# arielmission-space/PAOS

Hardware: AMD Instinct MI355X
Metric: wavefronts/sec (4096^2 c128, 20-surface chain) + achieved HBM GB/s (higher is better)
Workload: dtype c128 (f64); 1 GPU; SYN20 20-surface chain (SURVEY 8d: 43 2-D FFTs per wavefront as the reference runs it), 4096x4096 fp64, walked 512-wavelength sweep, 32 wavefronts/GPU/step, PSFs stay in HBM; separable pass programs + ptp identities ([24] passes/wavefront, parity 1e-15..2e-14 vs oracle); grid=4096, batch_per_gpu=32, parallelism=wavefront-sharded x1, transport=none (single process), ranks_seen=1, launcher=none

## Files before the change

include/paos_hip.h:

```cpp
#ifndef PAOS_HIP_H
#define PAOS_HIP_H

#ifdef __cplusplus
extern "C" {
#endif

typedef struct paos_ctx paos_ctx;

enum { PAOS_OK = 0, PAOS_EINVAL = 1, PAOS_EHIP = 2, PAOS_EUNSUPPORTED = 3 };
enum { PAOS_F64 = 0, PAOS_F32 = 1 };
enum { PAOS_SHAPE_ELLIPSE = 0, PAOS_SHAPE_RECT = 1 };
enum { PAOS_KERNEL_PASS_ROWS = 0, PAOS_KERNEL_PASS_COLS = 1, PAOS_KERNEL_PASS_ANY = 2 };
enum { PAOS_PW_SIGN = 1, PAOS_PW_QPHASE_CENTRED = 2, PAOS_PW_QPHASE_NATURAL = 3, PAOS_PW_SCALE = 4,
       PAOS_PW_MASK = 5 };
enum { PAOS_PWF_MUL2PI = 1,
       PAOS_PWF_X_ONLY = 2, PAOS_PWF_Y_ONLY = 4 };
enum { PAOS_MAX_PW = 6 };
enum { PAOS_NORM_SLOTS = 64 };
enum { PAOS_WHAT_FIELD = 0, PAOS_WHAT_AMPLITUDE = 1, PAOS_WHAT_PHASE = 2, PAOS_WHAT_INTENSITY = 3 };

enum { PAOS_PHASE_STRIDE = 5 };
enum { PAOS_APERTURE_STRIDE = 8 };
enum { PAOS_ZERNIKE_HEAD = 8 };

// ... 68 lines not shown
int paos_phase_map_items(paos_ctx* ctx, const double* host_wfe, unsigned long long key, int n_items, const double* items,
                         const double* wl);
int paos_psd_screen(paos_ctx* ctx, const double* host_noise, const double* host_rough, const double* params,
                    unsigned long long key, double* host_out);
int paos_ptp(paos_ctx* ctx, const double* params);
int paos_stw(paos_ctx* ctx, const double* params, int inverse);
int paos_wts(paos_ctx* ctx, const double* params, int inverse);
int paos_focus_begin(paos_ctx* ctx);
int paos_focus_plane(paos_ctx* ctx, const double* params);
int paos_focus_end(paos_ctx* ctx);
enum { PAOS_OTF_MTF = 0, PAOS_OTF_COMPLEX = 1 };
int paos_otf_compute(paos_ctx* ctx);
int paos_otf_fetch(paos_ctx* ctx, int item, int what, void* host_out);
int paos_otf_cuts(paos_ctx* ctx, double* host_out);
int paos_blur_table(int n, double d, double sigma, double pixel, double* t);
enum { PAOS_BLUR_ITEM = 6 };
int paos_blur_apply(paos_ctx* ctx, const double* per_item);
enum { PAOS_EE_GIVEN = 0, PAOS_EE_CENTROID = 1, PAOS_EE_PEAK = 2 };
enum { PAOS_EE_ITEM = 4 };
enum { PAOS_EE_SUMMARY = 9 };
int paos_ee_compute(paos_ctx* ctx, int bins, int square, int centre_mode, const double* per_item);
int paos_ee_fetch(paos_ctx* ctx, double* summary, double* curves);
int paos_zoom_weights(int n, int s, double frac, double* w, int* carry);
enum { PAOS_ZOOM_PSF = 0, PAOS_ZOOM_FIELD = 1 };
int paos_zoom_compute(paos_ctx* ctx, int m, int s, const double* centres, int want_field);
int paos_zoom_tiles(int n, int batch, int m, int* pt_y, int* pt_x);
int paos_zoom_fetch(paos_ctx* ctx, int item, int what, void* host_out);
int paos_run_passes(paos_ctx* ctx, const paos_pass* passes, int n_passes, const double* blocks,
                    int n_blocks);
int paos_copy_yardstick(paos_ctx* ctx, int reps, double* ms_per_launch, double* bytes_per_launch);
int paos_record_set_stats(paos_ctx* ctx, unsigned long long* found, unsigned long long* rendered);
int paos_central_half_stats(paos_ctx* ctx, unsigned long long* central, unsigned long long* plain);
int paos_narrow_window_stats(paos_ctx* ctx, unsigned long long* narrow, unsigned long long* other);
int paos_frugal_built(int precision, int n, const int* record);
int paos_pass_builds(paos_ctx* ctx, int* records, int capacity, int* count);
int paos_deferred_stop_stats(paos_ctx* ctx, unsigned long long* rode, unsigned long long* settled);
int paos_ctx_set_pruning(paos_ctx* ctx, int on);
int paos_run_passes_live(paos_ctx* ctx, const paos_pass* passes, int n_passes, const double* blocks,
                         int n_blocks, const double* live_rows);
int paos_run_program(paos_ctx* ctx, const paos_pass* passes, int n_passes, const double* blocks, int n_blocks,
                     const paos_program_opts* opts);
int paos_zernike(paos_ctx* ctx, int nmax, int kdim, const double* table, const double* params,
                 int param_stride, double* host_wfe);
int paos_zernike_like(paos_ctx* ctx, int nmax, int kdim, const double* table, const double* params,
                      int param_stride, const double* same_as, double* host_wfe);


int paos_pupil_aperture(paos_ctx* ctx, int shape, const double* params);
int paos_pupil_upload(paos_ctx* ctx, int item, const double* host_weights);
int paos_zernike_gram(paos_ctx* ctx, int nmax, int kdim, const double* table, const double* params,
                      int param_stride, int K, const double* poly, int use_pupil, double* host_out);
int paos_zernike_pupil(paos_ctx* ctx, int nmax, int kdim, const double* table, const double* params,
                       int param_stride, double* host_wfe);

enum { PAOS_WF_UNIFORM = 0, PAOS_WF_INTENSITY = 1 };
enum { PAOS_WF_SUMMARY = 10 };
int paos_wavefront_fit(paos_ctx* ctx, int nmax, int kdim, const double* table, const double* params, int param_stride,
                       int K, const double* poly, int weight_mode, int use_pupil, const double* min_intensity);
int paos_wavefront_fetch(paos_ctx* ctx, double* summary, double* sums);

enum { PAOS_DETECTOR_GEOM = 6 };
enum { PAOS_DETECTOR_ITEM = 3 };
enum { PAOS_DETECTOR_SCRATCH_MIB = 512 };
int paos_detector_begin(paos_ctx* ctx, const double* geom);
int paos_detector_add(paos_ctx* ctx, const double* per_item);
int paos_detector_images(paos_ctx* ctx, const double* per_item, double* host_out);
// ... 10 lines not shown
```

paos_amd/_lib.py:

```python
import ctypes
import os
import threading
import weakref

import numpy as np

_HERE = os.path.dirname(os.path.abspath(__file__))
LIB_PATH = os.environ.get("PAOS_LIB") or os.path.join(_HERE, "libpaoship.so")

PAOS_F64, PAOS_F32 = 0, 1
SHAPE_ELLIPSE, SHAPE_RECT = 0, 1
WHAT_FIELD, WHAT_AMPLITUDE, WHAT_PHASE, WHAT_INTENSITY = 0, 1, 2, 3
KERNEL_PASS_ROWS, KERNEL_PASS_COLS, KERNEL_PASS_ANY = 0, 1, 2
PW_SIGN, PW_QPHASE_CENTRED, PW_QPHASE_NATURAL, PW_SCALE, PW_MASK = 1, 2, 3, 4, 5
PWF_MUL2PI = 1
PWF_X_ONLY, PWF_Y_ONLY = 2, 4
MAX_PW = 6
OTF_MTF, OTF_COMPLEX = 0, 1
EE_GIVEN, EE_CENTROID, EE_PEAK = 0, 1, 2
EE_ITEM, EE_SUMMARY, EE_MAX_BINS = 4, 9, 1024
WF_UNIFORM, WF_INTENSITY = 0, 1
WF_SUMMARY, WF_MAX_TERMS = 10, 63
ZOOM_PSF, ZOOM_FIELD = 0, 1
ZOOM_MAX_TABLES = 256
# ... 47 lines not shown
    "paos_norm2": (ctypes.c_int, [_c_ctx, _dbl_p]),
    "paos_norm2_enqueue": (ctypes.c_int, [_c_ctx, ctypes.POINTER(ctypes.c_int)]),
    "paos_norm2_fetch": (ctypes.c_int, [_c_ctx, ctypes.c_int, _dbl_p]),
    "paos_norm2_release": (ctypes.c_int, [_c_ctx, ctypes.c_int]),
    "paos_psf_metrics": (ctypes.c_int, [_c_ctx, ctypes.c_int, _dbl_p, ctypes.c_double, ctypes.c_double, _dbl_p]),
    "paos_phase": (ctypes.c_int, [_c_ctx, _dbl_p, ctypes.c_int]),
    "paos_phase_map": (ctypes.c_int, [_c_ctx, ctypes.c_int, _dbl_p, ctypes.c_double]),
    "paos_ptp": (ctypes.c_int, [_c_ctx, _dbl_p]),
    "paos_stw": (ctypes.c_int, [_c_ctx, _dbl_p, ctypes.c_int]),
    "paos_wts": (ctypes.c_int, [_c_ctx, _dbl_p, ctypes.c_int]),
    "paos_focus_begin": (ctypes.c_int, [_c_ctx]),
    "paos_focus_plane": (ctypes.c_int, [_c_ctx, _dbl_p]),
    "paos_focus_end": (ctypes.c_int, [_c_ctx]),
    "paos_otf_compute": (ctypes.c_int, [_c_ctx]),
    "paos_otf_fetch": (ctypes.c_int, [_c_ctx, ctypes.c_int, ctypes.c_int, ctypes.c_void_p]),
    "paos_otf_cuts": (ctypes.c_int, [_c_ctx, _dbl_p]),
    "paos_blur_table": (ctypes.c_int, [ctypes.c_int, ctypes.c_double, ctypes.c_double, ctypes.c_double, _dbl_p]),
    "paos_blur_apply": (ctypes.c_int, [_c_ctx, _dbl_p]),
    "paos_ee_compute": (ctypes.c_int, [_c_ctx, ctypes.c_int, ctypes.c_int, ctypes.c_int, _dbl_p]),
    "paos_ee_fetch": (ctypes.c_int, [_c_ctx, _dbl_p, _dbl_p]),
    "paos_wavefront_fit": (ctypes.c_int, [_c_ctx, ctypes.c_int, ctypes.c_int, _dbl_p, _dbl_p, ctypes.c_int, ctypes.c_int, _dbl_p,
                                          ctypes.c_int, ctypes.c_int, _dbl_p]),
    "paos_wavefront_fetch": (ctypes.c_int, [_c_ctx, _dbl_p, _dbl_p]),
    "paos_zoom_weights": (ctypes.c_int, [ctypes.c_int, ctypes.c_int, ctypes.c_double, _dbl_p, ctypes.POINTER(ctypes.c_int)]),
    "paos_zoom_compute": (ctypes.c_int, [_c_ctx, ctypes.c_int, ctypes.c_int, _dbl_p, ctypes.c_int]),
    "paos_zoom_fetch": (ctypes.c_int, [_c_ctx, ctypes.c_int, ctypes.c_int, ctypes.c_void_p]),
    "paos_zoom_tiles": (ctypes.c_int, [ctypes.c_int, ctypes.c_int, ctypes.c_int, ctypes.POINTER(ctypes.c_int),
                                       ctypes.POINTER(ctypes.c_int)]),
    "paos_run_passes": (ctypes.c_int, [_c_ctx, ctypes.POINTER(Pass), ctypes.c_int, _dbl_p, ctypes.c_int]),
    "paos_copy_yardstick": (ctypes.c_int, [_c_ctx, ctypes.c_int, _dbl_p, _dbl_p]),
    "paos_record_set_stats": (ctypes.c_int, [_c_ctx, ctypes.POINTER(ctypes.c_ulonglong), ctypes.POINTER(ctypes.c_ulonglong)]),
    "paos_central_half_stats": (ctypes.c_int, [_c_ctx, ctypes.POINTER(ctypes.c_ulonglong), ctypes.POINTER(ctypes.c_ulonglong)]),
    "paos_narrow_window_stats": (ctypes.c_int, [_c_ctx, ctypes.POINTER(ctypes.c_ulonglong), ctypes.POINTER(ctypes.c_ulonglong)]),
    "paos_frugal_built": (ctypes.c_int, [ctypes.c_int, ctypes.c_int, ctypes.POINTER(ctypes.c_int)]),
    "paos_pass_builds": (ctypes.c_int, [_c_ctx, ctypes.POINTER(ctypes.c_int), ctypes.c_int, ctypes.POINTER(ctypes.c_int)]),
    "paos_deferred_stop_stats": (ctypes.c_int, [_c_ctx, ctypes.POINTER(ctypes.c_ulonglong), ctypes.POINTER(ctypes.c_ulonglong)]),
    "paos_ctx_set_pruning": (ctypes.c_int, [_c_ctx, ctypes.c_int]),
    "paos_run_passes_live": (ctypes.c_int, [_c_ctx, ctypes.POINTER(Pass), ctypes.c_int, _dbl_p, ctypes.c_int, _dbl_p]),
    "paos_zernike": (ctypes.c_int, [_c_ctx, ctypes.c_int, ctypes.c_int, _dbl_p, _dbl_p, ctypes.c_int, _dbl_p]),
    "paos_psf_keep": (ctypes.c_int, [_c_ctx]),
    "paos_psf_keep_power": (ctypes.c_int, [_c_ctx, ctypes.POINTER(ctypes.c_int)]),
    "paos_psf_fetch": (ctypes.c_int, [_c_ctx, ctypes.c_int, _dbl_p]),
    "paos_host_alloc": (ctypes.c_int, [ctypes.c_ulonglong, ctypes.POINTER(ctypes.c_void_p)]),
    "paos_host_free": (ctypes.c_int, [ctypes.c_void_p]),
    "paos_export_pinned": (ctypes.c_int, [_c_ctx, ctypes.c_int, ctypes.c_int, ctypes.c_void_p]),
    "paos_start": (ctypes.c_int, [_c_ctx, ctypes.c_double, ctypes.c_double, ctypes.c_int, _dbl_p, _dbl_p]),
    "paos_pupil_aperture": (ctypes.c_int, [_c_ctx, ctypes.c_int, _dbl_p]),
    "paos_pupil_upload": (ctypes.c_int, [_c_ctx, ctypes.c_int, _dbl_p]),
    "paos_zernike_like": (ctypes.c_int, [_c_ctx, ctypes.c_int, ctypes.c_int, _dbl_p, _dbl_p, ctypes.c_int, _dbl_p, _dbl_p]),
    "paos_zernike_gram": (ctypes.c_int, [_c_ctx, ctypes.c_int, ctypes.c_int, _dbl_p, _dbl_p, ctypes.c_int,
                                         ctypes.c_int, _dbl_p, ctypes.c_int, _dbl_p]),
    "paos_zernike_pupil": (ctypes.c_int, [_c_ctx, ctypes.c_int, ctypes.c_int, _dbl_p, _dbl_p, ctypes.c_int, _dbl_p]),
    "paos_start_rows": (ctypes.c_int, [_c_ctx, ctypes.c_double, ctypes.c_double, ctypes.c_int, _dbl_p, _dbl_p, _dbl_p]),
    "paos_zero_outside_rows": (ctypes.c_int, [_c_ctx, _dbl_p]),
    "paos_phase_map_items": (ctypes.c_int, [_c_ctx, _dbl_p, ctypes.c_ulonglong, ctypes.c_int, _dbl_p, _dbl_p]),
    "paos_psd_screen": (ctypes.c_int, [_c_ctx, _dbl_p, _dbl_p, _dbl_p, ctypes.c_ulonglong, _dbl_p]),
    "paos_start_box": (ctypes.c_int, [_c_ctx, ctypes.c_double, ctypes.c_double, ctypes.c_int, _dbl_p, _dbl_p, _dbl_p, _dbl_p]),
    "paos_start_zernike_box": (ctypes.c_int, [_c_ctx, ctypes.c_double, ctypes.c_double, ctypes.c_int, _dbl_p, _dbl_p, _dbl_p, _dbl_p,
                                              ctypes.c_int, ctypes.c_int, _dbl_p, _dbl_p, ctypes.c_int, ctypes.POINTER(ctypes.c_int)]),
    "paos_zero_outside_box": (ctypes.c_int, [_c_ctx, _dbl_p, _dbl_p]),
    "paos_norm2_enqueue_box": (ctypes.c_int, [_c_ctx, _dbl_p, _dbl_p, _dbl_p, ctypes.POINTER(ctypes.c_int)]),
    "paos_norm2_enqueue_rows": (ctypes.c_int, [_c_ctx, _dbl_p, ctypes.POINTER(ctypes.c_int)]),
    "paos_norm2_enqueue_rows_like": (ctypes.c_int, [_c_ctx, _dbl_p, _dbl_p, ctypes.POINTER(ctypes.c_int)]),
    "paos_run_program": (ctypes.c_int, [_c_ctx, ctypes.POINTER(Pass), ctypes.c_int, _dbl_p, ctypes.c_int,
                                        ctypes.POINTER(ProgramOpts)]),
    "paos_detector_begin": (ctypes.c_int, [_c_ctx, _dbl_p]),
# ... 557 lines not shown
        ctr = None if centres is None else zoom_centres(centres, self.batch, self.n)
        zoom_check(size, oversample, self.n)
        self._check(self._lib.paos_zoom_compute(self._ctx, int(size), int(oversample), _dptr(ctr) if ctr is not None else None,
                                                1 if field else 0), "paos_zoom_compute")
        self._zoom_size = int(size)

    def zoom_fetch(self, item=0, what="psf"):
        if what not in ("psf", "field"):
            raise ValueError(f"what must be 'psf' or 'field', got {what!r}")
        m = getattr(self, "_zoom_size", 1)
        out = np.empty((m, m), dtype=np.float64 if what == "psf" else np.complex128)
        self._check(self._lib.paos_zoom_fetch(self._ctx, int(item), ZOOM_PSF if what == "psf" else ZOOM_FIELD,
                                              out.ctypes.data_as(ctypes.c_void_p)), "paos_zoom_fetch")
        return out

    def copy_yardstick(self, reps=10):
        ms, nbytes = ctypes.c_double(0.0), ctypes.c_double(0.0)
        self._check(self._lib.paos_copy_yardstick(self._ctx, int(reps), ctypes.byref(ms), ctypes.byref(nbytes)),
                    "paos_copy_yardstick")
        return ms.value, nbytes.value

    def record_set_stats(self):
        found, rendered = ctypes.c_ulonglong(0), ctypes.c_ulonglong(0)
        self._check(self._lib.paos_record_set_stats(self._ctx, ctypes.byref(found), ctypes.byref(rendered)),
                    "paos_record_set_stats")
        return int(found.value), int(rendered.value)

    def central_half_stats(self):
        central, plain = ctypes.c_ulonglong(0), ctypes.c_ulonglong(0)
        self._check(self._lib.paos_central_half_stats(self._ctx, ctypes.byref(central), ctypes.byref(plain)),
                    "paos_central_half_stats")
        return int(central.value), int(plain.value)

    def pass_builds(self, capacity=64):
        count = ctypes.c_int(0)
        buf = (ctypes.c_int * (9 * capacity))()
        self._check(self._lib.paos_pass_builds(self._ctx, buf, capacity, ctypes.byref(count)), "paos_pass_builds")
        if count.value > capacity:
            return self.pass_builds(count.value)
        return [tuple(buf[9 * i:9 * i + 9]) for i in range(count.value)]

    def deferred_stop_stats(self):
        rode, settled = ctypes.c_ulonglong(0), ctypes.c_ulonglong(0)
        self._check(self._lib.paos_deferred_stop_stats(self._ctx, ctypes.byref(rode), ctypes.byref(settled)),
                    "paos_deferred_stop_stats")
        return int(rode.value), int(settled.value)

    def set_pruning(self, on):
        self._check(self._lib.paos_ctx_set_pruning(self._ctx, 1 if on else 0), "paos_ctx_set_pruning")

    def run_passes(self, passes, blocks, live_rows=None, rows_stale=False, final_intensity=False, live_cols=None):
        b = np.ascontiguousarray(blocks, dtype=np.float64)
        if b.ndim != 3 or b.shape[1:] != (self.batch, PHASE_STRIDE):
            raise ValueError("blocks must be [n_blocks][batch][5]")
        arr = (Pass * len(passes))()
        for dst, src in zip(arr, passes):
            dst.axis, dst.fft1, dst.fft2 = src["axis"], src.get("fft1", -1), src.get("fft2", -1)
            for name in ("pre", "mid", "post"):
                ops = src.get(name, ())
                if len(ops) > MAX_PW:
                    raise ValueError("too many operators in one pass slot")
                setattr(dst, "n_" + name, len(ops))
                lst = getattr(dst, name)
                for i, (kind, flags, block) in enumerate(ops):
                    lst[i].kind, lst[i].flags, lst[i].block = kind, flags, block
        if rows_stale or final_intensity:
# ... 104 lines not shown
```

paos_amd/csrc/context.hip:

```cpp
#include "host.h"

#include <cmath>
#include <complex>
#include <cstdio>
#include <cstring>
#include <mutex>
#include <set>
#include <utility>

namespace {

thread_local std::string g_err;

}

int fail(paos_ctx* c, int code, const std::string& msg) {
  if (c) c->err = msg;
  g_err = msg;
  return code;
}

namespace {

bool dump_arena() {
// ... 358 lines not shown
  if (n > capacity) return fail(c, PAOS_EINVAL, "profile buffer too small");
  for (int i = 0; i < n; ++i) lines_out[i] = (size_t)i < c->prof_lines.size() ? c->prof_lines[i] : 0.0;
  *count = n;
  return PAOS_OK;
}

int paos_profile_end(paos_ctx* c, int* launches, double* total_ms) {
  return profile_end(c, launches, total_ms, nullptr, nullptr);
}

int paos_profile_end_split(paos_ctx* c, int* launches, double* total_ms, int* pruned_launches, double* pruned_ms) {
  if (!pruned_launches || !pruned_ms) return fail(c, PAOS_EINVAL, "null argument");
  return profile_end(c, launches, total_ms, pruned_launches, pruned_ms);
}

int paos_ctx_destroy(paos_ctx* c) {
  if (!c) return PAOS_OK;
  (void)hipSetDevice(c->device);
  if (c->stream) (void)hipStreamSynchronize(c->stream);
  for (hipEvent_t e : c->prof_events) (void)hipEventDestroy(e);
  if (c->field) (void)hipFree(c->field);
  if (c->tw) (void)hipFree(c->tw);
  if (c->staging) (void)hipFree(c->staging);
  if (c->tables) (void)hipFree(c->tables);
  if (c->mask) (void)hipFree(c->mask);
  if (c->metric_partial) (void)hipFree(c->metric_partial);
  if (c->metric_out) (void)hipFree(c->metric_out);
  if (c->metric_host) (void)hipHostFree(c->metric_host);
  for (auto& ms : c->mask_sets) {
    if (ms.lines) (void)hipFree(ms.lines);
    if (ms.vals) (void)hipFree(ms.vals);
  }
  if (c->mask_overflow) (void)hipFree(c->mask_overflow);
  if (c->partial) (void)hipFree(c->partial);
  if (c->norm2) (void)hipFree(c->norm2);
  if (c->norm2_host) (void)hipHostFree(c->norm2_host);
  if (c->psf) (void)hipFree(c->psf);
  if (c->focus_spec) (void)hipFree(c->focus_spec);
  if (c->otf_spec) (void)hipFree(c->otf_spec);
  if (c->otf_cuts) (void)hipFree(c->otf_cuts);
  if (c->zoom_t) (void)hipFree(c->zoom_t);
  if (c->zoom_psf) (void)hipFree(c->zoom_psf);
  if (c->zoom_field) (void)hipFree(c->zoom_field);
  if (c->zoom_tabs) (void)hipFree(c->zoom_tabs);
  if (c->map_dev) (void)hipFree(c->map_dev);
  if (c->psd_scratch) (void)hipFree(c->psd_scratch);
  if (c->start_norm2) (void)hipFree(c->start_norm2);
  if (c->start_partial) (void)hipFree(c->start_partial);
  if (c->psd_bad) (void)hipFree(c->psd_bad);
  if (c->pow_partial) (void)hipFree(c->pow_partial);
  if (c->dyn_scale) (void)hipFree(c->dyn_scale);
  if (c->ptab) (void)hipFree(c->ptab);
  if (c->psf_partial) (void)hipFree(c->psf_partial);
  if (c->det_img) (void)hipFree(c->det_img);
  if (c->det_rows) (void)hipFree(c->det_rows);
  if (c->det_out) (void)hipFree(c->det_out);
  if (c->ee_buf) (void)hipFree(c->ee_buf);
  if (c->wf_buf) (void)hipFree(c->wf_buf);
  for (int i = 0; i < 2; ++i) {
    if (c->bounce[i]) (void)hipHostFree(c->bounce[i]);
    if (c->bounce_ev[i]) (void)hipEventDestroy(c->bounce_ev[i]);
  }
  if (c->arena.host) (void)hipHostFree(c->arena.host);
  if (c->arena.dev) (void)hipFree(c->arena.dev);
  for (int k = 0; k < kArenaSlabs; ++k)
    if (c->arena.fence[k]) (void)hipEventDestroy(c->arena.fence[k]);
// ... 34 lines not shown
  HIPCHK(c, hipStreamSynchronize(c->stream));
  c->norm_busy[ticket] = false;
  std::memcpy(host_out, c->norm2_host + (size_t)ticket * c->batch, (size_t)c->batch * sizeof(double));
  return check_mask_overflow(c);
}

int paos_norm2_release(paos_ctx* c, int ticket) {
  if (!c || ticket < 0 || ticket >= kNormSlots) return fail(c, PAOS_EINVAL, "bad ticket");
  c->norm_busy[ticket] = false;
  return PAOS_OK;
}

int paos_record_set_stats(paos_ctx* c, unsigned long long* found, unsigned long long* rendered) {
  if (!c || !found || !rendered) return fail(c, PAOS_EINVAL, "bad record-set request");
  *found = c->mask_hits;
  *rendered = c->mask_rendered;
  return PAOS_OK;
}

int paos_central_half_stats(paos_ctx* c, unsigned long long* central, unsigned long long* plain) {
  if (!c || !central || !plain) return fail(c, PAOS_EINVAL, "bad central-half request");
  *central = c->central_launches;
  *plain = c->plain_launches;
  return PAOS_OK;
}

int paos_narrow_window_stats(paos_ctx* c, unsigned long long* narrow, unsigned long long* other) {
  if (!c || !narrow || !other) return fail(c, PAOS_EINVAL, "bad narrow-window request");
  *narrow = c->narrow_launches;
  *other = c->other_launches;
  return PAOS_OK;
}

int paos_deferred_stop_stats(paos_ctx* c, unsigned long long* rode, unsigned long long* settled) {
  if (!c || !rode || !settled) return fail(c, PAOS_EINVAL, "bad deferred-stop request");
  *rode = c->deferred_rode;
  *settled = c->deferred_settled;
  return PAOS_OK;
}

int paos_ctx_set_pruning(paos_ctx* c, int on) {
  if (!c) return fail(c, PAOS_EINVAL, "null context");
  c->prune = on != 0;
  return PAOS_OK;
}

}
```

paos_amd/csrc/host.h:

```cpp
#pragma once
#include "../../include/paos_hip.h"

#include <hip/hip_runtime.h>

#include <cstdlib>
#include <string>
#include <type_traits>
#include <vector>

#include "arena_layout.h"
#include "frugal_pass.h"
#include "pass_records.h"

using namespace paos;

#ifndef PAOS_BR
#define PAOS_BR 4
#endif
#ifndef PAOS_PAD_BLOCKS
#define PAOS_PAD_BLOCKS 3
#endif
inline constexpr int BR = PAOS_BR;
#ifndef PAOS_F32_BR
#define PAOS_F32_BR 8
// ... 74 lines not shown
  bool ee_computed = false, ee_valid = false;
  double* wf_buf = nullptr;
  size_t wf_bytes = 0;
  int wf_pairs = 0;
  bool wf_fitted = false;
  void* bounce[2] = {nullptr, nullptr};
  hipEvent_t bounce_ev[2] = {nullptr, nullptr};
  void* field = nullptr;
  void* tw = nullptr;
  void* staging = nullptr;
  cx<double>* tables = nullptr;
  double* mask = nullptr;
  double* metric_partial = nullptr;
  double* metric_out = nullptr;
  double* metric_host = nullptr;
  struct MaskSet {
    MaskLine* lines = nullptr;
    double* vals = nullptr;
    std::vector<double> key;
    unsigned long long used = 0;
    int line_lo = 0, line_hi = 0;
  };
  static constexpr int kMaskSets = 8;
  MaskSet mask_sets[kMaskSets];
  unsigned long long mask_clock = 0;
  unsigned long long mask_hits = 0, mask_rendered = 0;
  size_t lds_pad = 0;
  bool central_half = true;
  unsigned long long central_launches = 0, plain_launches = 0;
  bool narrow_windows = true;
  unsigned long long narrow_launches = 0, other_launches = 0;
  std::vector<int> pass_builds;
  int* mask_overflow = nullptr;
  double* partial = nullptr;
  double* norm2 = nullptr;
  double* norm2_host = nullptr;
  bool prune = true;
  int norm_slot = 0;
  bool norm_busy[64] = {};
  int nparts = 0;
  Arena arena;
  std::string err;
  int prof_kind = -1;
  std::vector<hipEvent_t> prof_events;
  std::vector<int> prof_tags;
  int prof_next_tag = 0;
  double prof_next_bytes = 0.0;
  std::vector<double> prof_bytes;
  double prof_next_lines = 0.0;
  std::vector<double> prof_lines;
  size_t prof_used = 0;
};

#pragma GCC visibility push(hidden)

int fail(paos_ctx* c, int code, const std::string& msg);

#define HIPCHK(c, call)                                                                     \
  do {                                                                                      \
    hipError_t e_ = (call);                                                                 \
    if (e_ != hipSuccess)                                                                   \
      return fail((c), PAOS_EHIP,                                                           \
                  std::string(#call) + ": " + hipGetErrorString(e_) + " (" __FILE__ ":" +   \
                      std::to_string(__LINE__) + ")");                                      \
  } while (0)

// ... 129 lines not shown
```

paos_amd/csrc/paos_hip.hip:

```cpp
#include "host.h"

#include <algorithm>
#include <cmath>
#include <cstring>

#include "item_groups.h"
#include "pointwise.h"

namespace {

int pw_blocks(const paos_ctx* c) {
  const size_t total = (size_t)c->item_stride;
  size_t b = (total + kPwThreads - 1) / kPwThreads;
  return (int)(b < 2048 ? b : 2048);
}

__global__ void dyn_scale_set_kernel(double* dyn, const double* norm2, const double* enable, int batch) {
  const int i = blockIdx.x * blockDim.x + threadIdx.x;
  if (i < batch) dyn[i] = (!enable || enable[i] != 0.0) ? 1.0 / sqrt(norm2[i]) : 1.0;
}
__global__ void dyn_scale_reset_kernel(double* dyn, int batch) {
  const int i = blockIdx.x * blockDim.x + threadIdx.x;
  if (i < batch) dyn[i] = 1.0;
}
// ... 8 lines not shown
}

}

int dyn_scale_reset(paos_ctx* c) {
  hipLaunchKernelGGL(dyn_scale_reset_kernel, dim3((c->batch + 255) / 256), dim3(256), 0, c->stream, c->dyn_scale, c->batch);
  HIPCHK(c, hipGetLastError());
  c->dyn_pending = false;
  return PAOS_OK;
}

int settle_scale(paos_ctx* c, bool field_is_overwritten) {
  if (!c->dyn_pending) return PAOS_OK;
  ++c->deferred_settled;
  if (!field_is_overwritten) {
    const dim3 grid(pw_blocks(c), c->batch), block(kPwThreads);
    dispatch_layout(c, [&](auto t, auto) {
      using T = decltype(t);
      hipLaunchKernelGGL(scale_by_kernel<T>, grid, block, 0, c->stream, (cx<T>*)c->field, c->dyn_scale, c->item_stride);
    });
  }
  return dyn_scale_reset(c);
}

static_assert(kMaskRenders == kMaskJobs, "a call's renderings go out in one launch per shape");
int render_mask_records(paos_ctx* c, const MaskRender* renders, int count) {
  MaskJobs jobs{};
  for (int j = 0; j < count; ++j) {
    const MaskRender& r = renders[j];
    const paos_ctx::MaskSet& ms = c->mask_sets[r.set];
    jobs.job[j] = MaskJob{r.params, r.shared, ms.lines, ms.vals, r.axis, r.line0, r.line_end, r.shapes};
  }
  jobs.batch_stride = c->batch * (int)FP_STRIDE; jobs.param_stride = (int)FP_STRIDE; jobs.n = c->n; jobs.overflow = c->mask_overflow;
  {
    const int mode = mask_render_mode();
    jobs.windows = mode != 0 ? 1 : 0;
    jobs.pairs = mode >= 2 ? mode - 1 : 0;
    jobs.rect_blocks = mask_rect_blocks() ? 1 : 0;
  }
  int widest = 0, shapes = 0;
  for (int j = 0; j < count; ++j) {
    widest = std::max(widest, jobs.job[j].line_end - jobs.job[j].line0);
    shapes |= jobs.job[j].shapes;
  }
  const dim3 block(256);
  const int per_wg = 4 * (jobs.pairs >= 2 ? 4 : (jobs.pairs ? 2 : 1));
  if (shapes & 1) hipLaunchKernelGGL(mask_lines_kernel<0>, dim3((widest + per_wg - 1) / per_wg, c->batch, count), block, 0, c->stream, jobs);
  const int rect_per_wg = 4 * (jobs.rect_blocks ? 64 : 1);
  if (shapes & 2) hipLaunchKernelGGL(mask_lines_kernel<1>, dim3((widest + rect_per_wg - 1) / rect_per_wg, c->batch, count), block, 0, c->stream, jobs);
  HIPCHK(c, hipGetLastError());
  return PAOS_OK;
}

int render_mask_weights(paos_ctx* c, const double* ap) {
  if (!c->mask) HIPCHK(c, hipMalloc(&c->mask, (size_t)c->batch * c->item_stride * sizeof(double)));
  const dim3 grid(pw_blocks(c), c->batch), block(kPwThreads);
  const double* ap2 = ap + (size_t)c->batch * FP_STRIDE;
  dispatch_layout(c, [&](auto t, auto br) {
    using T = decltype(t);
    constexpr int BRV = decltype(br)::value;
    hipLaunchKernelGGL((aperture_kernel<T, BRV, Lay<T>::BC, 0>), grid, block, 0, c->stream, (cx<T>*)nullptr, ap, ap2, FP_STRIDE, c->n, c->pitch, c->item_stride, c->mask, 1);
    hipLaunchKernelGGL((aperture_kernel<T, BRV, Lay<T>::BC, 1>), grid, block, 0, c->stream, (cx<T>*)nullptr, ap, ap2, FP_STRIDE, c->n, c->pitch, c->item_stride, c->mask, 1);
  });
  HIPCHK(c, hipGetLastError());
  return PAOS_OK;
}

int pointwise_pass(paos_ctx* c, const PassArgs& a) {
  const dim3 grid(pw_blocks(c), c->batch), block(kPwThreads);
  dispatch_layout(c, [&](auto t, auto br) {
    hipLaunchKernelGGL((pointwise_kernel<decltype(t), decltype(br)::value, Lay<decltype(t)>::BC>), grid, block, 0, c->stream, a, c->n);
  });
  HIPCHK(c, hipGetLastError());
  return PAOS_OK;
}

namespace {

const char* const kPhaseMapOverflow = "the phase argument 2 pi w / wl of the map's largest value is not finite";
bool phase_map_argument_finite(double wmax, double wl) { return std::isfinite((6.283185307179586 * wmax) / wl); }
// ... 951 lines not shown
```

paos_amd/csrc/passes.hip:

```cpp
#include "frugal_launch.h"

#include <algorithm>
#include <cmath>
#include <cstdio>
#include <cstring>

#include "pass_program.h"
#include "phase_tables.h"

namespace {

int check_ops(paos_ctx* c, const paos_pw_op* ops, int count, int n_blocks) {
  if (count < 0 || count > PAOS_MAX_PW) return fail(c, PAOS_EINVAL, "too many pointwise operators in a pass");
  for (int o = 0; o < count; ++o) {
    if (ops[o].kind < PAOS_PW_SIGN || ops[o].kind > PAOS_PW_MASK) return fail(c, PAOS_EINVAL, "unknown pointwise operator");
    if (ops[o].block < 0 || ops[o].block >= n_blocks) return fail(c, PAOS_EINVAL, "operator block index out of range");
    if (ops[o].kind == PAOS_PW_MASK && ops[o].block + 1 >= n_blocks) return fail(c, PAOS_EINVAL, "an aperture operator needs two parameter blocks");
  }
  return PAOS_OK;
}

bool use_tables() {
  static const bool on = env_is("PAOS_PHASE_TABLES", '1');
  return on;
}

bool use_frugal() {
  static const bool on = !env_is("PAOS_NO_FRUGAL", '1');
  return on;
}

bool frugal_sizes(const paos_ctx* c) {
  return use_frugal() && c->n >= (c->precision == PAOS_F64 ? 1024 : 2048);
}

int ensure_mask_store(paos_ctx* c) {
  if (!c->mask_overflow) {
    HIPCHK(c, hipMalloc(&c->mask_overflow, sizeof(int)));
    HIPCHK(c, hipMemsetAsync(c->mask_overflow, 0, sizeof(int), c->stream));
  }
  return PAOS_OK;
}

int assign_mask_set(paos_ctx* c, const paos_pass& p, LoweredPass& lp, const double* blocks) {
  std::vector<double> key;
  key.reserve((size_t)2 * c->batch * FP_STRIDE + c->batch + 3);
  key.push_back((double)p.axis);
  key.push_back((double)(mask_render_mode() + (mask_rect_blocks() ? 0 : 8)));
  const double* ap = blocks + (size_t)lp.mask_block * c->batch * FP_STRIDE;
  key.insert(key.end(), ap, ap + (size_t)2 * c->batch * FP_STRIDE);
  key.insert(key.end(), lp.mask_shared.begin(), lp.mask_shared.end());
  int hit = -1, victim = 0;
  for (int k = 0; k < paos_ctx::kMaskSets; ++k) {
    const paos_ctx::MaskSet& ms = c->mask_sets[k];
    if (!ms.key.empty() && ms.key.size() == key.size() && !std::memcmp(ms.key.data(), key.data(), key.size() * sizeof(double))) hit = k;
    if (ms.used < c->mask_sets[victim].used) victim = k;
  }
  const int k = hit >= 0 ? hit : victim;
  paos_ctx::MaskSet& ms = c->mask_sets[k];
  if (!ms.lines) {
    for (paos_ctx::MaskSet& m2 : c->mask_sets) {
      if (m2.lines) continue;
      HIPCHK(c, hipMalloc(&m2.lines, (size_t)c->batch * c->n * sizeof(MaskLine)));
      HIPCHK(c, hipMalloc(&m2.vals, (size_t)c->batch * c->n * 2 * kMaskW * sizeof(double)));
    }
  }
  ms.used = ++c->mask_clock;
  lp.mask_set = k;
  lp.mask_render = hit < 0;
  lp.mask_shapes = 0;
  for (int it = 0; it < c->batch; ++it) {
    const double* a1 = ap + (size_t)it * FP_STRIDE;
// ... 391 lines not shown
  return take_power_ticket(c, c->psf_partial, c->n / frugal_tile_lines(c, r.passes[r.n_passes - 1].axis), nullptr, final_ticket);
}

int run_passes_impl(paos_ctx* c, const paos_pass* passes, int n_passes, const double* blocks, int n_blocks,
                    const double* entry_rows, bool entry_stale, int* final_ticket, int final_mode, const double* entry_cols) {
  int rc = validate_program(c, passes, n_passes, blocks, n_blocks, final_ticket);
  if (rc) return rc;
  final_mode = final_ticket ? (final_mode == 2 ? 2 : 1) : 0;
  ProgramRun r(c, passes, n_passes, blocks, n_blocks);
  if ((rc = open_batch(r)) || (rc = lower_and_assign_sets(r)) || (rc = settle_stop(r))) return rc;
  plan_lines(r, entry_rows, entry_stale, entry_cols);
  if (entry_stale && entry_rows && entry_zero_first(r.d, r.pruned, r.low, entry_rows, entry_cols)) {
    if ((rc = entry_cols ? zero_outside_box(c, entry_rows, entry_cols) : zero_outside_rows(c, entry_rows))) return rc;
  }
  if ((rc = prepare_store(r, final_mode)) || (rc = batch_renderings(r)) || (rc = plan_and_stage_launches(r))) return rc;
  if ((rc = r.ab.commit())) return rc;
  for (size_t at = 0; at < r.renderings.size(); at += kMaskRenders)
    if ((rc = render_mask_records(c, r.renderings.data() + at, (int)std::min<size_t>(kMaskRenders, r.renderings.size() - at)))) return rc;
  if ((rc = launch_staged_tables(c, r.staged)) || (rc = launch_chunks(r))) return rc;
  return final_mode ? hand_out_ticket(r, final_mode, final_ticket) : PAOS_OK;
}

}

int run_passes(paos_ctx* c, const paos_pass* passes, int n_passes, const double* blocks, int n_blocks, const double* entry_rows,
               bool entry_stale, int* final_ticket, int final_mode, const double* entry_cols) {
  const int rc = arena_settled(c, run_passes_impl(c, passes, n_passes, blocks, n_blocks, entry_rows, entry_stale, final_ticket, final_mode, entry_cols));
  if (rc != PAOS_OK && c) forget_mask_sets(c);
  return rc;
}

int mask_render_mode() {
  if (env_is("PAOS_MASK_SCAN", '1')) return 0;
  return env_is("PAOS_MASK_PAIRS", '0') ? 1 : (env_is("PAOS_MASK_PAIRS", '1') ? 2 : 3);
}
bool mask_rect_blocks() {
  return !env_is("PAOS_MASK_RECT_BLOCKS", '0');
}

namespace {

struct Program {
  std::vector<paos_pass> passes;
  std::vector<double> blocks;
  int batch;
  explicit Program(int b) : batch(b) {}
  int add_block(const double* src, double v1, double v2, double v3, double v4, bool copy) {
    const int id = (int)(blocks.size() / ((size_t)batch * FP_STRIDE));
    for (int i = 0; i < batch; ++i) {
      const double* s = src + (size_t)i * FP_STRIDE;
      if (copy) blocks.insert(blocks.end(), s, s + FP_STRIDE);
      else blocks.insert(blocks.end(), {s[FP_ENABLE], v1, v2, v3, v4});
    }
    return id;
  }
  paos_pass& add_pass(int axis, int fft1, int fft2) {
    paos_pass p{};
    p.axis = axis; p.fft1 = fft1; p.fft2 = fft2;
    passes.push_back(p);
    return passes.back();
  }
};
void push(paos_pw_op* list, int& count, int kind, int block, int flags = 0) { list[count++] = {kind, flags, block}; }

enum FftOp { OP_PTP, OP_STW, OP_WTS };

int fft_op(paos_ctx* c, FftOp op, const double* params, int inverse) {
// ... 103 lines not shown
```

paos_amd/csrc/pointwise.h:

```cpp
#pragma once
#include "frugal_pass.h"
#include "item_window.h"
#include "pointwise_shared.h"

namespace paos {

template <typename T>
__global__ void fill_kernel(cx<T>* f, size_t total, T re, T im) {
  size_t i = (size_t)blockIdx.x * blockDim.x + threadIdx.x;
  for (; i < total; i += (size_t)gridDim.x * blockDim.x) f[i] = {re, im};
}

template <typename T>
__global__ void rmw_copy_kernel(cx<T>* f, size_t total) {
  size_t i = (size_t)blockIdx.x * blockDim.x + threadIdx.x;
  for (; i < total; i += (size_t)gridDim.x * blockDim.x) {
    cx<T> v = f[i];
    asm volatile("" : "+v"(v.x), "+v"(v.y));
    f[i] = v;
  }
}

template <typename T, int BR, int BC>
__global__ void import_kernel(cx<T>* f, const cx<double>* staged, int n, unsigned pitch) {
  const size_t total = (size_t)pitch * (n / BR);
  size_t m = (size_t)blockIdx.x * blockDim.x + threadIdx.x;
  for (; m < total; m += (size_t)gridDim.x * blockDim.x) {
    int r, c;
    if (!layout_unmap<BR, BC>(m, n, pitch, r, c)) continue;
    const cx<double> v = staged[(size_t)r * n + c];
    f[m] = {(T)v.x, (T)v.y};
  }
}

template <typename T, int BR, int BC>
__global__ void export_kernel(const cx<T>* f, double* out, int n, unsigned pitch, int what) {
// ... 816 lines not shown
  }
  const int len0 = e.p1 - e.p0, len1 = e.p3 - e.p2i;
  for (unsigned long long todo = in_lines; todo; todo &= todo - 1) {
    const int k = (int)__ffsll((long long)todo) - 1;
    double* vout = jb.vals + ((size_t)item * n + (first + k)) * (2 * kMaskW);
    for (int j = lane; j < len0; j += 64) vout[j] = prof[j];
    for (int j = lane; j < len1; j += 64) vout[kMaskW + j] = prof[kMaskW + j];
  }
}

template <int SHAPE>
__global__ void __launch_bounds__(kMaskWaves * 64) mask_lines_kernel(MaskJobs jobs) {
  const MaskJob& jb = jobs.job[blockIdx.z];
  if (!(jb.shapes & (1 << SHAPE))) return;
  const int item = blockIdx.y;
  if (jb.shared[item] != 0.0) return;
  const int lane = threadIdx.x & 63;
  const int wave = blockIdx.x * (blockDim.x >> 6) + (threadIdx.x >> 6);
  if (SHAPE == 1 && jobs.rect_blocks != 0) {
    __shared__ double prof[kMaskWaves][2 * kMaskW];
    mask_rect_block_render(jobs, jb, item, jb.line0 + 64 * wave, lane, prof[threadIdx.x >> 6]);
    return;
  }
  const int per = SHAPE == 0 && jobs.pairs != 0 ? (jobs.pairs >= 2 ? 4 : 2) : 1;
  const int first = jb.line0 + per * wave;
  if (first >= jb.line_end || first >= jobs.n) return;
  if (SHAPE == 0 && per == 4 && mask_multi_render<4>(jobs, jb, item, first, lane)) return;
  for (int f = first; f < first + per; f += 2) {
    if (SHAPE == 0 && per >= 2 && mask_multi_render<2>(jobs, jb, item, f, lane)) continue;
    for (int line = f; line < f + (per >= 2 ? 2 : 1); ++line) {
      if (SHAPE == 0 && jobs.windows != 0 && mask_multi_render<1>(jobs, jb, item, line, lane)) continue;
      mask_line_render<SHAPE>(jobs, jb, item, line, lane);
    }
  }
}


template <int NMAXC>
__device__ __forceinline__ double zernike_wfe(const double* table, const double* coef_c, const double* coef_s, int nmax, int kdim,
                                              double x, double y, double rr, double rho, bool origin_y, double co, double so) {
  double wfe = 0.0;
  double c1 = 1.0, s1 = 0.0;
  if (rr > 0.0) {
    c1 = (origin_y ? y : x) / rr;
    s1 = (origin_y ? x : y) / rr;
  }
  const double cr = c1 * co - s1 * so, sr = s1 * co + c1 * so;
  const double xj = 1.0 - 2.0 * rho * rho;
  double rho_pow = 1.0, cm = 1.0, sm = 0.0;
  auto order = [&](int am, int k_end) __attribute__((always_inline)) {
    double pkm1 = 0.0, pk = 1.0;
    for (int k = 0; k <= k_end; ++k) {
      if (k > 0) {
        const double* abc = table + ((size_t)am * kdim + k) * 3;
        const double pn = (abc[0] * xj + abc[1]) * pk - abc[2] * pkm1;
        pkm1 = pk;
        pk = pn;
      }
      const size_t ci = (size_t)am * kdim + k;
      wfe += (rho_pow * pk) * (coef_c[ci] * cm + coef_s[ci] * sm);
    }
    rho_pow *= rho;
    const double cn = cm * cr - sm * sr;
    sm = sm * cr + cm * sr;
    cm = cn;
  };
// ... 313 lines not shown
```

Before: 2496 wavefronts/s.

## Render ellipse mask records per 64-line block with shared undecided-pixel list

Adds a default-on mask_blocks_kernel in which each wavefront handles 64 lines at once. Each lane classifies its line's edge-window pixels as in, out or undecided. The undecided pixels from all lanes are compacted into a shared-memory list so that the expensive per-pixel weight evaluation runs lane-parallel across the whole block instead of per line. Lines that overflow the list or have no fitting window fall back to the existing per-line renderers. Device atomic counters and a stats API are added, which brings extra atomics, LDS use and complexity.

```diff
diff --git a/include/paos_hip.h b/include/paos_hip.h
--- a/include/paos_hip.h
+++ b/include/paos_hip.h
@@ -124,6 +124,7 @@
 int paos_record_set_stats(paos_ctx* ctx, unsigned long long* found, unsigned long long* rendered);
 int paos_central_half_stats(paos_ctx* ctx, unsigned long long* central, unsigned long long* plain);
 int paos_narrow_window_stats(paos_ctx* ctx, unsigned long long* narrow, unsigned long long* other);
+int paos_record_block_stats(paos_ctx* ctx, unsigned long long* out);
 int paos_frugal_built(int precision, int n, const int* record);
 int paos_pass_builds(paos_ctx* ctx, int* records, int capacity, int* count);
 int paos_deferred_stop_stats(paos_ctx* ctx, unsigned long long* rode, unsigned long long* settled);
diff --git a/paos_amd/_lib.py b/paos_amd/_lib.py
--- a/paos_amd/_lib.py
+++ b/paos_amd/_lib.py
@@ -103,6 +103,7 @@
     "paos_record_set_stats": (ctypes.c_int, [_c_ctx, ctypes.POINTER(ctypes.c_ulonglong), ctypes.POINTER(ctypes.c_ulonglong)]),
     "paos_central_half_stats": (ctypes.c_int, [_c_ctx, ctypes.POINTER(ctypes.c_ulonglong), ctypes.POINTER(ctypes.c_ulonglong)]),
     "paos_narrow_window_stats": (ctypes.c_int, [_c_ctx, ctypes.POINTER(ctypes.c_ulonglong), ctypes.POINTER(ctypes.c_ulonglong)]),
+    "paos_record_block_stats": (ctypes.c_int, [_c_ctx, ctypes.POINTER(ctypes.c_ulonglong)]),
     "paos_frugal_built": (ctypes.c_int, [ctypes.c_int, ctypes.c_int, ctypes.POINTER(ctypes.c_int)]),
     "paos_pass_builds": (ctypes.c_int, [_c_ctx, ctypes.POINTER(ctypes.c_int), ctypes.c_int, ctypes.POINTER(ctypes.c_int)]),
     "paos_deferred_stop_stats": (ctypes.c_int, [_c_ctx, ctypes.POINTER(ctypes.c_ulonglong), ctypes.POINTER(ctypes.c_ulonglong)]),
@@ -726,6 +727,11 @@
                     "paos_central_half_stats")
         return int(central.value), int(plain.value)
 
+    def record_block_stats(self):
+        out = (ctypes.c_ulonglong * 3)()
+        self._check(self._lib.paos_record_block_stats(self._ctx, out), "paos_record_block_stats")
+        return int(out[0]), int(out[1]), int(out[2])
+
     def pass_builds(self, capacity=64):
         count = ctypes.c_int(0)
         buf = (ctypes.c_int * (9 * capacity))()
diff --git a/paos_amd/csrc/context.hip b/paos_amd/csrc/context.hip
--- a/paos_amd/csrc/context.hip
+++ b/paos_amd/csrc/context.hip
@@ -414,6 +414,7 @@
     if (ms.vals) (void)hipFree(ms.vals);
   }
   if (c->mask_overflow) (void)hipFree(c->mask_overflow);
+  if (c->block_stats) (void)hipFree(c->block_stats);
   if (c->partial) (void)hipFree(c->partial);
   if (c->norm2) (void)hipFree(c->norm2);
   if (c->norm2_host) (void)hipHostFree(c->norm2_host);
@@ -514,6 +515,15 @@
   return PAOS_OK;
 }
 
+int paos_record_block_stats(paos_ctx* c, unsigned long long* out) {
+  if (!c || !out) return fail(c, PAOS_EINVAL, "bad record-block request");
+  out[0] = out[1] = out[2] = 0ull;
+  if (!c->block_stats) return PAOS_OK;
+  HIPCHK(c, hipStreamSynchronize(c->stream));
+  HIPCHK(c, hipMemcpy(out, c->block_stats, 3 * sizeof(unsigned long long), hipMemcpyDeviceToHost));
+  return PAOS_OK;
+}
+
 int paos_deferred_stop_stats(paos_ctx* c, unsigned long long* rode, unsigned long long* settled) {
   if (!c || !rode || !settled) return fail(c, PAOS_EINVAL, "bad deferred-stop request");
   *rode = c->deferred_rode;
diff --git a/paos_amd/csrc/host.h b/paos_amd/csrc/host.h
--- a/paos_amd/csrc/host.h
+++ b/paos_amd/csrc/host.h
@@ -130,6 +130,7 @@
   unsigned long long narrow_launches = 0, other_launches = 0;
   std::vector<int> pass_builds;
   int* mask_overflow = nullptr;
+  unsigned long long* block_stats = nullptr;
   double* partial = nullptr;
   double* norm2 = nullptr;
   double* norm2_host = nullptr;
diff --git a/paos_amd/csrc/paos_hip.hip b/paos_amd/csrc/paos_hip.hip
--- a/paos_amd/csrc/paos_hip.hip
+++ b/paos_amd/csrc/paos_hip.hip
@@ -64,12 +64,10 @@
     jobs.job[j] = MaskJob{r.params, r.shared, ms.lines, ms.vals, r.axis, r.line0, r.line_end, r.shapes};
   }
   jobs.batch_stride = c->batch * (int)FP_STRIDE; jobs.param_stride = (int)FP_STRIDE; jobs.n = c->n; jobs.overflow = c->mask_overflow;
-  {
-    const int mode = mask_render_mode();
-    jobs.windows = mode != 0 ? 1 : 0;
-    jobs.pairs = mode >= 2 ? mode - 1 : 0;
-    jobs.rect_blocks = mask_rect_blocks() ? 1 : 0;
-  }
+  const int mode = mask_render_mode();
+  jobs.windows = mode != 0 ? 1 : 0;
+  jobs.pairs = mode >= 2 ? std::min(mode, 3) - 1 : 0;
+  jobs.rect_blocks = mask_rect_blocks() ? 1 : 0;
   int widest = 0, shapes = 0;
   for (int j = 0; j < count; ++j) {
     widest = std::max(widest, jobs.job[j].line_end - jobs.job[j].line0);
@@ -77,7 +75,11 @@
   }
   const dim3 block(256);
   const int per_wg = 4 * (jobs.pairs >= 2 ? 4 : (jobs.pairs ? 2 : 1));
-  if (shapes & 1) hipLaunchKernelGGL(mask_lines_kernel<0>, dim3((widest + per_wg - 1) / per_wg, c->batch, count), block, 0, c->stream, jobs);
+  constexpr int block_per_wg = kMaskBlockLines * kMaskWaves;
+  if ((shapes & 1) && mode == 4)
+    hipLaunchKernelGGL(mask_blocks_kernel, dim3((widest + block_per_wg - 1) / block_per_wg, c->batch, count), block, 0, c->stream, jobs, c->block_stats);
+  else if (shapes & 1)
+    hipLaunchKernelGGL(mask_lines_kernel<0>, dim3((widest + per_wg - 1) / per_wg, c->batch, count), block, 0, c->stream, jobs);
   const int rect_per_wg = 4 * (jobs.rect_blocks ? 64 : 1);
   if (shapes & 2) hipLaunchKernelGGL(mask_lines_kernel<1>, dim3((widest + rect_per_wg - 1) / rect_per_wg, c->batch, count), block, 0, c->stream, jobs);
   HIPCHK(c, hipGetLastError());
diff --git a/paos_amd/csrc/passes.hip b/paos_amd/csrc/passes.hip
--- a/paos_amd/csrc/passes.hip
+++ b/paos_amd/csrc/passes.hip
@@ -38,6 +38,10 @@
   if (!c->mask_overflow) {
     HIPCHK(c, hipMalloc(&c->mask_overflow, sizeof(int)));
     HIPCHK(c, hipMemsetAsync(c->mask_overflow, 0, sizeof(int), c->stream));
+  }
+  if (!c->block_stats) {
+    HIPCHK(c, hipMalloc(&c->block_stats, 3 * sizeof(unsigned long long)));
+    HIPCHK(c, hipMemsetAsync(c->block_stats, 0, 3 * sizeof(unsigned long long), c->stream));
   }
   return PAOS_OK;
 }
@@ -495,7 +499,9 @@
 
 int mask_render_mode() {
   if (env_is("PAOS_MASK_SCAN", '1')) return 0;
-  return env_is("PAOS_MASK_PAIRS", '0') ? 1 : (env_is("PAOS_MASK_PAIRS", '1') ? 2 : 3);
+  if (env_is("PAOS_MASK_PAIRS", '0')) return 1;
+  if (env_is("PAOS_MASK_PAIRS", '1')) return 2;
+  return env_is("PAOS_MASK_BLOCKS", '0') ? 3 : 4;
 }
 bool mask_rect_blocks() {
   return !env_is("PAOS_MASK_RECT_BLOCKS", '0');
diff --git a/paos_amd/csrc/pointwise.h b/paos_amd/csrc/pointwise.h
--- a/paos_amd/csrc/pointwise.h
+++ b/paos_amd/csrc/pointwise.h
@@ -2,6 +2,7 @@
 #include "frugal_pass.h"
 #include "item_window.h"
 #include "pointwise_shared.h"
+#include "record_blocks.h"
 
 namespace paos {
 
@@ -884,6 +885,111 @@
       if (SHAPE == 0 && jobs.windows != 0 && mask_multi_render<1>(jobs, jb, item, line, lane)) continue;
       mask_line_render<SHAPE>(jobs, jb, item, line, lane);
     }
+  }
+}
+
+constexpr int kMaskBlockLines = 64;
+__global__ void __launch_bounds__(kMaskWaves * 64) mask_blocks_kernel(MaskJobs jobs, unsigned long long* stats) {
+  const MaskJob& jb = jobs.job[blockIdx.z];
+  if (!(jb.shapes & 1)) return;
+  const int item = blockIdx.y;
+  if (jb.shared[item] != 0.0) return;
+  const int lane = threadIdx.x & 63, wv = threadIdx.x >> 6;
+  const int n = jobs.n, axis = jb.axis;
+  const int first = jb.line0 + kMaskBlockLines * (blockIdx.x * kMaskWaves + wv);
+  if (first >= jb.line_end || first >= n) return;
+  MaskLineGeom<0> g;
+  if (!g.init(jobs, jb, item)) return;
+  __shared__ unsigned long long list_all[kMaskWaves][kBlockListCap];
+  __shared__ int counts_all[kMaskWaves][64];
+  unsigned long long* list = list_all[wv];
+  int* counts = counts_all[wv];
+  const auto wave_sync = [] {
+    __builtin_amdgcn_fence(__ATOMIC_RELEASE, "wavefront");
+    __builtin_amdgcn_wave_barrier();
+    __builtin_amdgcn_fence(__ATOMIC_ACQUIRE, "wavefront");
+  };
+
+  const int line = first + lane;
+  const bool valid = lane < kMaskBlockLines && line < jb.line_end && line < n;
+  const bool in_box = valid && g.in_box(axis, line);
+  int W = 0, wl0 = 0, wr0 = 0;
+  if (in_box) {
+    if (window_fit<8, 1>(g, axis, line, n, wl0, wr0)) W = 8;
+    else if (window_fit<16, 3>(g, axis, line, n, wl0, wr0)) W = 16;
+    else if (window_fit<32, 3>(g, axis, line, n, wl0, wr0)) W = 32;
+  }
+  unsigned long long in_bits = 0ull, und_bits = 0ull;
+  if (W != 0) {
+    const double sa = axis == 0 ? g.a : g.b, sc = axis == 0 ? g.b : g.a;
+    const double ca = axis == 0 ? g.xc : g.yc, cc = axis == 0 ? g.yc : g.xc;
+    const double lo_c = __dsub_rn((double)line - 0.5, cc), hi_c = __dsub_rn((double)line + 0.5, cc);
+    const double vv_lo = edge_square(lo_c, sc), vv_hi = edge_square(hi_c, sc);
+    unsigned in_l, in_r, und_l, und_r;
+    window_classes(wl0, W, ca, sa, lo_c, hi_c, vv_lo, vv_hi, in_l, und_l);
+    window_classes(wr0, W, ca, sa, lo_c, hi_c, vv_lo, vv_hi, in_r, und_r);
+    in_bits = (unsigned long long)in_l | ((unsigned long long)in_r << W);
+    und_bits = (unsigned long long)und_l | ((unsigned long long)und_r << W);
+  }
+  const int count = __popcll(und_bits);
+  counts[lane] = count;
+  wave_sync();
+  int offset, total;
+  list_layout(counts, 64, lane, offset, total);
+  const bool kept = W != 0 && list_keeps(offset, count);
+  if (kept) list_write(list, lane, offset, und_bits);
+  wave_sync();
+  for (int base = 0; base < total; base += 64) {
+    const int at = base + lane;
+    const unsigned long long e = at < total ? list[at] : 0ull;
+    const int owner = entry_line(e), k = entry_pixel(e);
+    const int oW = __shfl(W, owner), owl0 = __shfl(wl0, owner), owr0 = __shfl(wr0, owner);
+    if (at < total) list[at] = (unsigned long long)__double_as_longlong(line_weight(g, axis, first + owner, k < oW ? owl0 + k : owr0 + (k - oW)));
+  }
+  wave_sync();
+  if (valid && !in_box) jb.lines[(size_t)item * n + line] = {0, 0, 0, 0, 1.0, 0.0};
+  if (kept) {
+    unsigned long long not_out = in_bits, is_in = in_bits;
+    int at = offset;
+    for (unsigned long long m = und_bits; m; m &= m - 1, ++at) {
+      const double w = __longlong_as_double((long long)list[at]);
+      const unsigned long long bit = 1ull << __builtin_ctzll(m);
+      if (w != g.w_out) not_out |= bit;
+      if (w == g.w_in) is_in |= bit;
+    }
+    const unsigned long long win = (1ull << W) - 1ull;
+    const unsigned no_l = (unsigned)(not_out & win), no_r = (unsigned)((not_out >> W) & win), ii_l = (unsigned)(is_in & win), ii_r = (unsigned)((is_in >> W) & win);
+    LineExtents e = W == 8 ? extents_from_windows<8>(no_l, no_r, ii_l, ii_r, wl0, wr0, n)
+                           : (W == 16 ? extents_from_windows<16>(no_l, no_r, ii_l, ii_r, wl0, wr0, n) : extents_from_windows<32>(no_l, no_r, ii_l, ii_r, wl0, wr0, n));
+    close_record(e, jobs.overflow, true);
+    double* vout = jb.vals + ((size_t)item * n + line) * (2 * kMaskW);
+    for (int side = 0; side < 2; ++side) {
+      const int lo = side == 0 ? e.p0 : e.p2i, hi = side == 0 ? e.p1 : e.p3;
+      for (int pos = lo; pos < hi; ++pos) {
+        const int k = pos >= wl0 && pos < wl0 + W ? pos - wl0 : (pos >= wr0 && pos < wr0 + W ? W + pos - wr0 : -1);
+        if (k < 0) continue;
+        const unsigned long long below = und_bits & ((1ull << k) - 1ull);
+        const double w = (und_bits >> k) & 1ull ? __longlong_as_double((long long)list[offset + __popcll(below)]) : ((in_bits >> k) & 1ull ? g.w_in : g.w_out);
+        vout[side * kMaskW + pos - lo] = w;
+      }
+    }
+    jb.lines[(size_t)item * n + line] = {e.p0, e.p1, e.p2i, e.p3, 1.0, 0.0};
+  }
+  unsigned long long handed = __ballot(in_box && !kept);
+  {
+    const unsigned long long nk = __ballot(kept);
+    const unsigned long long add = lane == 0 ? (unsigned long long)__popcll(nk) : (lane == 1 ? (unsigned long long)__popcll(handed) : (unsigned long long)total);
+    if (lane < 3 && add != 0ull) atomicAdd(stats + lane, add);
+  }
+  while (handed) {
+    const int l = (int)__ffsll((long long)handed) - 1;
+    handed &= handed - 1;
+    if (jobs.pairs != 0 && l < 63 && ((handed >> (l + 1)) & 1ull) && mask_multi_render<2>(jobs, jb, item, first + l, lane)) {
+      handed &= handed - 1;
+      continue;
+    }
+    if (jobs.windows != 0 && mask_multi_render<1>(jobs, jb, item, first + l, lane)) continue;
+    mask_line_render<0>(jobs, jb, item, first + l, lane);
   }
 }
 
diff --git a/paos_amd/csrc/record_blocks.h b/paos_amd/csrc/record_blocks.h
--- /dev/null
+++ b/paos_amd/csrc/record_blocks.h
@@ -0,0 +1,63 @@
+#pragma once
+
+#if defined(__HIPCC__)
+#define PAOS_BLOCK_FN __host__ __device__ __forceinline__
+#else
+#define PAOS_BLOCK_FN inline
+#endif
+
+namespace paos {
+
+enum : int { kPixelOut = 0, kPixelIn = 1, kPixelUndecided = 2 };
+
+PAOS_BLOCK_FN double edge_square(double offset, double semi_axis) {
+  const double u = offset / semi_axis;
+  return u * u;
+}
+
+PAOS_BLOCK_FN int pixel_class(double lo_a, double hi_a, double uu_lo, double uu_hi, double lo_c, double hi_c, double vv_lo, double vv_hi) {
+  if (uu_lo + vv_lo <= 1.0 && uu_hi + vv_lo <= 1.0 && uu_lo + vv_hi <= 1.0 && uu_hi + vv_hi <= 1.0) return kPixelIn;
+  const double nu = lo_a > 0.0 ? uu_lo : (hi_a < 0.0 ? uu_hi : 0.0);
+  const double nv = lo_c > 0.0 ? vv_lo : (hi_c < 0.0 ? vv_hi : 0.0);
+  return nu + nv > 1.0 + 1.0e-9 ? kPixelOut : kPixelUndecided;
+}
+
+PAOS_BLOCK_FN void window_classes(int w0, int W, double centre, double semi_axis, double lo_c, double hi_c, double vv_lo, double vv_hi,
+                                  unsigned& in, unsigned& undecided) {
+  in = undecided = 0u;
+  double lo_a = ((double)w0 - 0.5) - centre, uu_lo = edge_square(lo_a, semi_axis);
+  for (int k = 0; k < W; ++k) {
+    const double hi_a = ((double)(w0 + k) + 0.5) - centre, uu_hi = edge_square(hi_a, semi_axis);
+    const int cls = pixel_class(lo_a, hi_a, uu_lo, uu_hi, lo_c, hi_c, vv_lo, vv_hi);
+    in |= (cls == kPixelIn ? 1u : 0u) << k;
+    undecided |= (cls == kPixelUndecided ? 1u : 0u) << k;
+    lo_a = hi_a; uu_lo = uu_hi;
+  }
+}
+
+constexpr int kBlockListCap = 1024;
+
+PAOS_BLOCK_FN void list_layout(const int* counts, int lines, int line, int& offset, int& total) {
+  int run = 0;
+  offset = total = 0;
+  for (int i = 0; i < lines; ++i) {
+    if (i == line) offset = run;
+    run += counts[i];
+    if (run <= kBlockListCap) total = run;
+  }
+}
+PAOS_BLOCK_FN bool list_keeps(int offset, int count) { return offset + count <= kBlockListCap; }
+
+PAOS_BLOCK_FN unsigned long long list_entry(int line, int pixel) { return ((unsigned long long)line << 6) | (unsigned long long)pixel; }
+PAOS_BLOCK_FN int entry_line(unsigned long long e) { return (int)(e >> 6); }
+PAOS_BLOCK_FN int entry_pixel(unsigned long long e) { return (int)(e & 63ull); }
+
+PAOS_BLOCK_FN int list_write(unsigned long long* list, int line, int offset, unsigned long long undecided) {
+  const int count = __builtin_popcountll(undecided);
+  if (!list_keeps(offset, count)) return 0;
+  int at = offset;
+  for (unsigned long long m = undecided; m; m &= m - 1) list[at++] = list_entry(line, __builtin_ctzll(m));
+  return count;
+}
+
+}
```

Measured after the change: 2539 wavefronts/s (median of 6 runs). 1.7% higher.
